# RaghuvirJonnagiri/LatticeBoltzmannSimulations

Measured on AMD Instinct MI355X. Metric: MLUPS (million lattice updates/sec) D2Q9 MRT cavity, higher is better.
Workload: dtype f32

## Files before the change

latticeboltzmannsimulations_amd/csrc/lbm_device.hpp:

```cpp
#pragma once
#include <hip/hip_runtime.h>

#include <type_traits>

#include "lbm_rheology.hpp"

namespace lbm {

constexpr int Q = 9;
constexpr int GH = 4;
constexpr int GHY = 10;

__host__ __device__ constexpr int cxk(int k) { return k == 1 || k == 5 || k == 8 ? 1 : (k == 3 || k == 6 || k == 7 ? -1 : 0); }
__host__ __device__ constexpr int cyk(int k) { return k == 2 || k == 5 || k == 6 ? 1 : (k == 4 || k == 7 || k == 8 ? -1 : 0); }

enum { SEM_PY = 0, SEM_GPU = 1, SEM_BB = 2, SEM_SOLID = 3 };
constexpr bool sem_is_bb(int sem) { return sem == SEM_BB || sem == SEM_SOLID; }
enum { C_SRT = 0, C_TRT = 1, C_MRT = 2,
       C_MRT_FAST = 3,
       C_SRT_FAST = 4,
       C_TRT_FAST = 5,
       C_SRT_PROM = 6, C_TRT_PROM = 7, C_MRT_PROM = 8 };
constexpr bool coll_is_mrt(int c) { return c == C_MRT || c == C_MRT_FAST || c == C_MRT_PROM; }
constexpr bool coll_is_fast(int c) { return c == C_MRT_FAST || c == C_SRT_FAST || c == C_TRT_FAST; }
constexpr bool coll_is_prom(int c) { return c == C_SRT_PROM || c == C_TRT_PROM || c == C_MRT_PROM; }

template <typename R>
struct Relax {
    R uLB, w_nu, w_m, w_e, w_eps, w_q;
};

typedef float f32x2 __attribute__((ext_vector_type(2)));
template <typename T> struct ScalarOf { typedef T type; };
template <> struct ScalarOf<f32x2> { typedef float type; };

template <int SEM>
__device__ __forceinline__ bool in_window(int k, int x, int gy, int X, int Y) {
    const int cx = cxk(k), cy = cyk(k);
    bool ok = true;
    if (sem_is_bb(SEM)) {
        return true;
    } else if (SEM == SEM_PY) {
        if (cx > 0) ok = ok && (x >= 1) && (x <= X - 2);
        if (cx < 0) ok = ok && (x <= X - 3);
        if (cy > 0) ok = ok && (gy <= Y - 3);
        if (cy < 0) ok = ok && (gy >= 1) && (gy <= Y - 2);
    } else {
        if (cx > 0) ok = ok && (x >= 1);
        if (cx < 0) ok = ok && (x <= X - 2);
        if (cy > 0) ok = ok && (gy <= Y - 2);
        if (cy < 0) ok = ok && (gy >= 1);
    }
    return ok;
}

template <typename T>
__device__ __forceinline__ T cu_of(int k, T ux, T uy) {
    switch (k) {
        case 1: return ux;
        case 2: return uy;
        case 3: return -ux;
        case 4: return -uy;
        case 5: return ux + uy;
        case 6: return -ux + uy;
        case 7: return -ux + -uy;
        case 8: return ux + -uy;
        default: return T{};
    }
}
template <typename R>
__device__ __forceinline__ R weight(int k) {
    return k == 0 ? (R)(4.0 / 9.0) : (k < 5 ? (R)(1.0 / 9.0) : (R)(1.0 / 36.));
}
template <bool FAST> __device__ __forceinline__ float div_(float a, float b) { return FAST ? a * __builtin_amdgcn_rcpf(b) : a / b; }
__device__ __forceinline__ double rcp_nr(double b) {
    double r = __builtin_amdgcn_rcp(b);
    r = __builtin_fma(__builtin_fma(-b, r, 1.0), r, r);
    r = __builtin_fma(__builtin_fma(-b, r, 1.0), r, r);
    return r;
}
template <bool FAST> __device__ __forceinline__ double div_(double a, double b) { return FAST ? a * rcp_nr(b) : a / b; }
template <bool FAST> __device__ __forceinline__ f32x2 div_(f32x2 a, f32x2 b) {
    return FAST ? a * f32x2{__builtin_amdgcn_rcpf(b.x), __builtin_amdgcn_rcpf(b.y)} : a / b;
}
template <bool FAST> __device__ __forceinline__ float sqrt_(float a) { return FAST ? __builtin_amdgcn_sqrtf(a) : sqrtf(a); }
template <bool FAST> __device__ __forceinline__ double sqrt_(double a) {
    if (!FAST) return sqrt(a);
    if (a <= 0.0) return 0.0;
    double y = __builtin_amdgcn_rsq(a);
    y = y * __builtin_fma(-0.5 * a * y, y, 1.5);
    y = y * __builtin_fma(-0.5 * a * y, y, 1.5);
    const double g = a * y;
    return __builtin_fma(__builtin_fma(-g, g, a), 0.5 * y, g);
}
template <bool FAST> __device__ __forceinline__ f32x2 sqrt_(f32x2 a) {
    return FAST ? f32x2{__builtin_amdgcn_sqrtf(a.x), __builtin_amdgcn_sqrtf(a.y)} : f32x2{sqrtf(a.x), sqrtf(a.y)};
}

template <typename F> __device__ __forceinline__ float lanes(F f, float a, float b) { return f(a, b); }
template <typename F> __device__ __forceinline__ f32x2 lanes(F f, f32x2 a, f32x2 b) { return f32x2{f(a.x, b.x), f(a.y, b.y)}; }
template <typename F> __device__ __forceinline__ float lanes(F f, float a, float b, float c) { return f(a, b, c); }
template <typename F> __device__ __forceinline__ f32x2 lanes(F f, f32x2 a, f32x2 b, f32x2 c) { return f32x2{f(a.x, b.x, c.x), f(a.y, b.y, c.y)}; }

__device__ __forceinline__ float feq_prom(float rt, float cu, float usqr) {
    const double c = (double)cu;
    return (float)((double)rt * (((1. + 3.0 * c) + (4.5 * c) * c) - 1.5 * (double)usqr));
}
__device__ __forceinline__ f32x2 feq_prom(f32x2 rt, f32x2 cu, f32x2 usqr) {
    return f32x2{feq_prom(rt.x, cu.x, usqr.x), feq_prom(rt.y, cu.y, usqr.y)};
}

template <typename T, bool PROM = false>
__device__ __forceinline__ void equ(T rho, T ux, T uy, T (&feq)[Q]) {
    typedef typename ScalarOf<T>::type S;
    const T usqr = ux * ux + uy * uy;
    if constexpr (PROM) {
#pragma unroll
        for (int k = 0; k < Q; ++k) feq[k] = feq_prom(rho * weight<S>(k), cu_of<T>(k, ux, uy), usqr);
        return;
    }
    const T c = (S)1.5 * usqr;
#pragma unroll
    for (int k = 0; k < Q; ++k) {
        const T cu = cu_of<T>(k, ux, uy);
        feq[k] = (rho * weight<S>(k)) * ((((S)1. + (S)3.0 * cu) + ((S)4.5 * cu) * cu) - c);
    }
}

template <typename R, bool FAST = false, int SEM = SEM_GPU>
__device__ __forceinline__ void macros(const R (&f)[Q], int x, int gy, int X, int Y, R uLB, R& rho, R& ux, R& uy) {
    rho = ((((((((f[0] + f[1]) + f[2]) + f[3]) + f[4]) + f[5]) + f[6]) + f[7]) + f[8]);
    ux = div_<FAST>((((((f[1] - f[3]) + f[5]) - f[6]) - f[7]) + f[8]), rho);
    uy = div_<FAST>((((((f[2] - f[4]) + f[5]) + f[6]) - f[7]) - f[8]), rho);
    if (sem_is_bb(SEM)) return;
    if (x == 0 || x == X - 1 || gy == Y - 1) { ux = (R)0; uy = (R)0; }
    if (gy == 0) {
        rho = ((f[0] + f[1]) + f[3]) + (R)2. * ((f[2] + f[5]) + f[6]);
        ux = uLB; uy = (R)0;
    }
}

__device__ __forceinline__ float fma_(float a, float b, float c) { return __builtin_fmaf(a, b, c); }
__device__ __forceinline__ double fma_(double a, double b, double c) { return __builtin_fma(a, b, c); }
__device__ __forceinline__ f32x2 fma_(f32x2 a, f32x2 b, f32x2 c) { return __builtin_elementwise_fma(a, b, c); }

template <typename T, int COLL, bool WM = false>
__device__ __forceinline__ void collide(const T (&f)[Q], T rho, const T (&feq)[Q],
                                        const Relax<typename ScalarOf<T>::type>& w, T w_nu, T (&out)[Q], bool lid = false, T w_m = T{}) {
    typedef typename ScalarOf<T>::type R;
    if (COLL == C_SRT || COLL == C_SRT_FAST || COLL == C_SRT_PROM) {
#pragma unroll
        for (int k = 0; k < Q; ++k) out[k] = f[k] - w_nu * (f[k] - feq[k]);
    } else if (COLL == C_TRT || COLL == C_TRT_FAST || COLL == C_TRT_PROM) {
        T fp[Q], fm[Q], ep[Q], em[Q];
        constexpr int pa[4] = {2, 5, 6, 1}, pb[4] = {4, 7, 8, 3};
#pragma unroll
        for (int i = 0; i < 4; ++i) {
            const int a = pa[i], b = pb[i];
            fp[a] = (R)0.5 * (f[a] + f[b]); fp[b] = fp[a];
            fm[a] = (R)0.5 * (f[a] - f[b]); fm[b] = -fm[a];
            ep[a] = (R)0.5 * (feq[a] + feq[b]); ep[b] = ep[a];
            em[a] = (R)0.5 * (feq[a] - feq[b]); em[b] = -em[a];
        }
        fp[0] = f[0]; fm[0] = T{}; ep[0] = feq[0]; em[0] = T{};
#pragma unroll
        for (int k = 0; k < Q; ++k) {
            if constexpr (WM) out[k] = (f[k] - w_nu * (fp[k] - ep[k])) - w_m * (fm[k] - em[k]);
            else out[k] = (f[k] - w_nu * (fp[k] - ep[k])) - w.w_m * (fm[k] - em[k]);
        }
    } else if (COLL == C_MRT_FAST) {
        const T a13 = f[1] + f[3], d13 = f[1] - f[3], a24 = f[2] + f[4], d24 = f[2] - f[4];
        const T a57 = f[5] + f[7], d57 = f[5] - f[7], a68 = f[6] + f[8], d68 = f[6] - f[8];
        const T sa = a13 + a24, sd = a57 + a68, dm = d57 - d68, dp = d57 + d68;
        const T r = (f[0] + sa) + sd;
        const T jx = d13 + dm, jy = d24 + dp;
        const T f04 = (R)4 * f[0];
        T e = fma_(T((R)2), sd, -sa) - f04;
        T eps = fma_(T((R)-2), sa, f04 + sd);
        T qx = fma_(T((R)-2), d13, dm), qy = fma_(T((R)-2), d24, dp);
        T pxx = a13 - a24, pxy = a57 - a68;
        const T jx2 = jx * jx, jy2 = jy * jy, j23 = (R)3 * (jx2 + jy2);
        const T rq = lid ? rho : r;
        e = fma_(T(-w.w_e), e - fma_(T((R)-2), rq, j23), e);
        eps = fma_(T(-w.w_eps), eps - fma_(T((R)9), jx2 * jy2, rq - j23), eps);
        qx = fma_(T(-w.w_q), qx - jx * fma_(T((R)3), jx2, T((R)-1)), qx);
        qy = fma_(T(-w.w_q), qy - jy * fma_(T((R)3), jy2, T((R)-1)), qy);
        pxx = fma_(-w_nu, pxx - (jx2 - jy2), pxx);
        pxy = fma_(-w_nu, fma_(-jx, jy, pxy), pxy);
        const R a9 = (R)(1.0 / 9), a36 = (R)(1.0 / 36), a18 = (R)(1.0 / 18), a6 = (R)(1.0 / 6),
                a12 = (R)(1.0 / 12), a4 = (R)(1.0 / 4);
        const T r9 = a9 * r;
        out[0] = a9 * ((r - e) + eps);
        const T A = fma_(T(-a18), eps, fma_(T(-a36), e, r9)), D = fma_(T(a36), eps, fma_(T(a18), e, r9));
        const T Ap = fma_(T(a4), pxx, A), Am = fma_(T(-a4), pxx, A), Dp = fma_(T(a4), pxy, D), Dm = fma_(T(-a4), pxy, D);
        const T bx = a6 * (jx - qx), by = a6 * (jy - qy);
        const T X = fma_(T(a12), qx, a6 * jx), Y = fma_(T(a12), qy, a6 * jy);
        const T XpY = X + Y, XmY = X - Y;
        out[1] = Ap + bx; out[3] = Ap - bx;
        out[2] = Am + by; out[4] = Am - by;
        out[5] = Dp + XpY; out[7] = Dp - XpY;
        out[8] = Dm + XmY; out[6] = Dm - XmY;
    } else {
        T m[Q], meq[Q];
        const T c2 = T((R)2), cm2 = T((R)-2);
        m[0] = (((((((f[0] + f[1]) + f[2]) + f[3]) + f[4]) + f[5]) + f[6]) + f[7]) + f[8];
        m[1] = fma_(c2, f[8], fma_(c2, f[7], fma_(c2, f[6], fma_(c2, f[5], ((((R)-4 * f[0] - f[1]) - f[2]) - f[3]) - f[4]))));
        m[2] = (((fma_(cm2, f[4], fma_(cm2, f[3], fma_(cm2, f[2], fma_(cm2, f[1], (R)4 * f[0])))) + f[5]) + f[6]) + f[7]) + f[8];
        m[3] = ((((f[1] - f[3]) + f[5]) - f[6]) - f[7]) + f[8];
        m[4] = (((fma_(c2, f[3], (R)-2 * f[1]) + f[5]) - f[6]) - f[7]) + f[8];
        m[5] = ((((f[2] - f[4]) + f[5]) + f[6]) - f[7]) - f[8];
        m[6] = (((fma_(c2, f[4], (R)-2 * f[2]) + f[5]) + f[6]) - f[7]) - f[8];
        m[7] = ((f[1] - f[2]) + f[3]) - f[4];
        m[8] = ((f[5] - f[6]) + f[7]) - f[8];
        const T jx = m[3], jy = m[5];
        meq[0] = rho;
        meq[1] = fma_(cm2, rho, (R)3.0 * (jx * jx + jy * jy));
        meq[2] = ((R)-3.0 * (jx * jx + jy * jy) + rho) + (R)9.0 * (((jx * jx) * jy) * jy);
        meq[3] = m[3];
        meq[4] = -jx + (R)3.0 * ((jx * jx) * jx);
        meq[5] = m[5];
        meq[6] = -jy + (R)3.0 * ((jy * jy) * jy);
        meq[7] = jx * jx - jy * jy;
        meq[8] = jx * jy;
        if constexpr (COLL == C_MRT_PROM) {
            const T s = jx * jx + jy * jy, p4 = ((jx * jx) * jy) * jy, x3 = (jx * jx) * jx, y3 = (jy * jy) * jy;
            meq[1] = lanes([](float r, float a) { return (float)(-2.0 * (double)r + 3.0 * (double)a); }, rho, s);
            meq[2] = lanes([](float a, float r, float b) { return (float)((-3.0 * (double)a + (double)r) + 9.0 * (double)b); }, s, rho, p4);
            meq[4] = lanes([](float j, float a) { return (float)((double)(-j) + 3.0 * (double)a); }, jx, x3);
            meq[6] = lanes([](float j, float a) { return (float)((double)(-j) + 3.0 * (double)a); }, jy, y3);
        }
        m[1] = m[1] - w.w_e * (m[1] - meq[1]);
        m[2] = m[2] - w.w_eps * (m[2] - meq[2]);
        m[4] = m[4] - w.w_q * (m[4] - meq[4]);
        m[6] = m[6] - w.w_q * (m[6] - meq[6]);
        m[7] = m[7] - w_nu * (m[7] - meq[7]);
        m[8] = m[8] - w_nu * (m[8] - meq[8]);
        const R a9 = (R)(1.0 / 9), a36 = (R)(1.0 / 36), a18 = (R)(1.0 / 18), a6 = (R)(1.0 / 6),
                a12 = (R)(1.0 / 12), a4 = (R)(1.0 / 4);
        const T q4 = T(a4), qm4 = T(-a4);
        out[0] = (a9 * m[0] + -a9 * m[1]) + a9 * m[2];
        out[1] = fma_(q4, m[7], (((a9 * m[0] + -a36 * m[1]) + -a18 * m[2]) + a6 * m[3]) + -a6 * m[4]);
        out[2] = fma_(qm4, m[7], (((a9 * m[0] + -a36 * m[1]) + -a18 * m[2]) + a6 * m[5]) + -a6 * m[6]);
        out[3] = fma_(q4, m[7], (((a9 * m[0] + -a36 * m[1]) + -a18 * m[2]) + -a6 * m[3]) + a6 * m[4]);
        out[4] = fma_(qm4, m[7], (((a9 * m[0] + -a36 * m[1]) + -a18 * m[2]) + -a6 * m[5]) + a6 * m[6]);
        out[5] = fma_(q4, m[8], (((((a9 * m[0] + a18 * m[1]) + a36 * m[2]) + a6 * m[3]) + a12 * m[4]) + a6 * m[5]) + a12 * m[6]);
        out[6] = fma_(qm4, m[8], (((((a9 * m[0] + a18 * m[1]) + a36 * m[2]) + -a6 * m[3]) + -a12 * m[4]) + a6 * m[5]) + a12 * m[6]);
        out[7] = fma_(q4, m[8], (((((a9 * m[0] + a18 * m[1]) + a36 * m[2]) + -a6 * m[3]) + -a12 * m[4]) + -a6 * m[5]) + -a12 * m[6]);
        out[8] = fma_(qm4, m[8], (((((a9 * m[0] + a18 * m[1]) + a36 * m[2]) + a6 * m[3]) + a12 * m[4]) + -a6 * m[5]) + -a12 * m[6]);
    }
}

constexpr int K_QEQ = Q;
constexpr int K_RHO = Q + 1;

template <typename T>
__device__ __forceinline__ T diag_flux(const T (&f)[Q]) {
    return -f[8] + (f[7] + (-f[6] + f[5]));
}
template <typename T, int COLL, bool TURB, bool WM = false>
__device__ __forceinline__ void equ_collide(const T (&g)[Q], T rho, T ux, T uy, const Relax<typename ScalarOf<T>::type>& w, T w_nu, T (&out)[Q], T& q2,
                                            bool lid = false, T w_m = T{}) {
    typedef typename ScalarOf<T>::type R;
    if constexpr ((COLL == C_SRT_FAST && !(TURB && sizeof(R) == 4)) || COLL == C_TRT_FAST) {
        const T base = fma_(T((R)-1.5), fma_(uy, uy, ux * ux), T((R)1));
        const T orho = w_nu * rho, c1 = (R)1 - w_nu;
        const T r1 = (R)(1.0 / 9) * orho, r5 = (R)(1.0 / 36) * orho;
        out[0] = fma_((R)(4.0 / 9) * orho, base, c1 * g[0]);
        if constexpr (COLL == C_SRT_FAST) {
            auto pair = [&](T cu, T rw, const T& ga, const T& gb, T& oa, T& ob) {
                const T e = fma_((R)4.5 * cu, cu, base), o = (R)3 * cu;
                oa = fma_(rw, e + o, c1 * ga);
                ob = fma_(rw, e - o, c1 * gb);
            };
            pair(ux, r1, g[1], g[3], out[1], out[3]);
            pair(uy, r1, g[2], g[4], out[2], out[4]);
            pair(ux + uy, r5, g[5], g[7], out[5], out[7]);
            pair(ux - uy, r5, g[8], g[6], out[8], out[6]);
        } else {
            const auto wm = [&] { if constexpr (WM) return w_m; else return w.w_m; }();
            const T mrho = wm * rho, hp = (R)0.5 * w_nu;
            const T m1 = (R)(1.0 / 9) * mrho, m5 = (R)(1.0 / 36) * mrho;
            const auto hm = (R)0.5 * wm;
            auto pair = [&](T cu, T rp, T rm, const T& ga, const T& gb, T& oa, T& ob) {
                const T e = fma_((R)4.5 * cu, cu, base), o = (R)3 * cu;
                const T P = fma_(-rp, e, hp * (ga + gb)), M = fma_(-rm, o, hm * (ga - gb));
                oa = (ga - P) - M;
                ob = (gb - P) + M;
            };
            pair(ux, r1, m1, g[1], g[3], out[1], out[3]);
            pair(uy, r1, m1, g[2], g[4], out[2], out[4]);
            pair(ux + uy, r5, m5, g[5], g[7], out[5], out[7]);
            pair(ux - uy, r5, m5, g[8], g[6], out[8], out[6]);
        }
        if (TURB) q2 = rho * (ux * uy);
    } else if constexpr (COLL == C_MRT_FAST) {
        T fe[Q];
        collide<T, COLL>(g, rho, fe, w, w_nu, out, lid);
        if (TURB) q2 = rho * (ux * uy);
    } else {
        T fe[Q];
        if (!coll_is_mrt(COLL) || TURB) equ<T, coll_is_prom(COLL)>(rho, ux, uy, fe);
        if constexpr (WM) collide<T, COLL, true>(g, rho, fe, w, w_nu, out, false, w_m);
        else collide<T, COLL>(g, rho, fe, w, w_nu, out);
        if (TURB) q2 = diag_flux<T>(fe);
    }
}

__device__ __forceinline__ float real_abs(float x) { return fabsf(x); }
__device__ __forceinline__ double real_abs(double x) { return fabs(x); }
__device__ __forceinline__ f32x2 real_abs(f32x2 x) { return f32x2{fabsf(x.x), fabsf(x.y)}; }

template <typename T, bool FAST = false, bool PROM = false>
__device__ __forceinline__ T smagorinsky_tau(const T (&f)[Q], T qeq_prev, T rho_prev, typename ScalarOf<T>::type omega) {
    typedef typename ScalarOf<T>::type R;
    const R tau0 = (R)1.0 / omega;
    const T q = diag_flux<T>(f) - qeq_prev;
    if constexpr (PROM) {
        const R tt = tau0 * tau0;
        return lanes([tau0, tt](float qq, float rp) {
            return (float)(0.5 * ((double)tau0 + sqrt((double)tt + (((18 * 1.4142) * (double)0.025f) * (double)fabsf(qq)) / (double)rp)));
        }, q, rho_prev);
    }
    return (R)0.5 * (tau0 + sqrt_<FAST>(tau0 * tau0 + div_<FAST>(((R)(18 * 1.4142) * (R)0.025) * real_abs(q), rho_prev)));
}
template <typename T, bool FAST = false, bool PROM = false>
__device__ __forceinline__ T smagorinsky_omega(const T (&f)[Q], T qeq_prev, T rho_prev, typename ScalarOf<T>::type omega) {
    typedef typename ScalarOf<T>::type R;
    return div_<FAST>(T((R)1.0), smagorinsky_tau<T, FAST, PROM>(f, qeq_prev, rho_prev, omega));
}

template <typename T, bool FAST = false, typename W = typename ScalarOf<T>::type>
__device__ __forceinline__ T subgrid_tau(const T (&f)[Q], T rho, T ux, T uy, W omega, typename ScalarOf<T>::type k) {
    typedef typename ScalarOf<T>::type R;
    const W tau0 = (R)1.0 / omega;
    const T sxx = ((((f[1] + f[3]) + f[5]) + f[6]) + f[7]) + f[8];
    const T syy = ((((f[2] + f[4]) + f[5]) + f[6]) + f[7]) + f[8];
    const T sxy = ((f[5] - f[6]) + f[7]) - f[8];
    const T r3 = rho * (R)(1.0 / 3), jx = rho * ux;
    const T pxx = sxx - (r3 + jx * ux);
    const T pyy = syy - (r3 + (rho * uy) * uy);
    const T pxy = sxy - jx * uy;
    const T n = sqrt_<FAST>((pxx * pxx + (R)2 * (pxy * pxy)) + pyy * pyy);
    return (R)0.5 * (tau0 + sqrt_<FAST>(tau0 * tau0 + div_<FAST>(k * n, rho)));
}
template <typename T, bool FAST = false, typename W = typename ScalarOf<T>::type>
__device__ __forceinline__ T subgrid_omega(const T (&f)[Q], T rho, T ux, T uy, W omega, typename ScalarOf<T>::type k) {
    typedef typename ScalarOf<T>::type R;
    return div_<FAST>(T((R)1.0), subgrid_tau<T, FAST, W>(f, rho, ux, uy, omega, k));
}

template <typename R>
struct Rheo {
    const R* tab;
    R inv_dg;
// ... 711 lines not shown
```

latticeboltzmannsimulations_amd/csrc/lbm_stream.hpp:

```cpp
#pragma once
#include "lbm_kernels.hpp"

constexpr int ST_WAVES = 16;
constexpr int ST_NT = ST_WAVES * 64;
constexpr int ST_MAX_S = ST_WAVES / 2;
constexpr int ST_LDS_BYTES = ST_WAVES * 9 * 1024;

__device__ __forceinline__ int dpp_from_lower(int v) { return __builtin_amdgcn_update_dpp(v, v, 0x138, 0xf, 0xf, false); }
__device__ __forceinline__ int dpp_from_upper(int v) { return __builtin_amdgcn_update_dpp(v, v, 0x130, 0xf, 0xf, false); }
__device__ __forceinline__ float lane_lower(float v) { return __builtin_bit_cast(float, dpp_from_lower(__builtin_bit_cast(int, v))); }
__device__ __forceinline__ float lane_upper(float v) { return __builtin_bit_cast(float, dpp_from_upper(__builtin_bit_cast(int, v))); }
__device__ __forceinline__ double lane_lower(double v) {
    const long long b = __builtin_bit_cast(long long, v);
    const unsigned lo = (unsigned)dpp_from_lower((int)(unsigned)b), hi = (unsigned)dpp_from_lower((int)(unsigned)(b >> 32));
    return __builtin_bit_cast(double, (long long)(((unsigned long long)hi << 32) | lo));
}
__device__ __forceinline__ double lane_upper(double v) {
    const long long b = __builtin_bit_cast(long long, v);
    const unsigned lo = (unsigned)dpp_from_upper((int)(unsigned)b), hi = (unsigned)dpp_from_upper((int)(unsigned)(b >> 32));
    return __builtin_bit_cast(double, (long long)(((unsigned long long)hi << 32) | lo));
}

__device__ __forceinline__ float lane_lower_e(float v, float edge) {
    return __builtin_bit_cast(float, __builtin_amdgcn_update_dpp(__builtin_bit_cast(int, edge), __builtin_bit_cast(int, v), 0x138, 0xf, 0xf, false));
}
__device__ __forceinline__ float lane_upper_e(float v, float edge) {
    return __builtin_bit_cast(float, __builtin_amdgcn_update_dpp(__builtin_bit_cast(int, edge), __builtin_bit_cast(int, v), 0x130, 0xf, 0xf, false));
}
__device__ __forceinline__ double lane_lower_e(double v, double edge) {
    const long long b = __builtin_bit_cast(long long, v), e = __builtin_bit_cast(long long, edge);
    const unsigned lo = (unsigned)__builtin_amdgcn_update_dpp((int)(unsigned)e, (int)(unsigned)b, 0x138, 0xf, 0xf, false);
    const unsigned hi = (unsigned)__builtin_amdgcn_update_dpp((int)(unsigned)(e >> 32), (int)(unsigned)(b >> 32), 0x138, 0xf, 0xf, false);
    return __builtin_bit_cast(double, (long long)(((unsigned long long)hi << 32) | lo));
}
__device__ __forceinline__ double lane_upper_e(double v, double edge) {
    const long long b = __builtin_bit_cast(long long, v), e = __builtin_bit_cast(long long, edge);
    const unsigned lo = (unsigned)__builtin_amdgcn_update_dpp((int)(unsigned)e, (int)(unsigned)b, 0x130, 0xf, 0xf, false);
    const unsigned hi = (unsigned)__builtin_amdgcn_update_dpp((int)(unsigned)(e >> 32), (int)(unsigned)(b >> 32), 0x130, 0xf, 0xf, false);
    return __builtin_bit_cast(double, (long long)(((unsigned long long)hi << 32) | lo));
}
template <typename R, int V>
__device__ __forceinline__ typename VecT<R, V>::type shift_from_lower_e(typename VecT<R, V>::type own, R edge) {
    typename VecT<R, V>::type r;
    r[0] = lane_lower_e(own[V - 1], edge);
#pragma unroll
    for (int c = 1; c < V; ++c) r[c] = own[c - 1];
    return r;
}
template <typename R, int V>
__device__ __forceinline__ typename VecT<R, V>::type shift_from_upper_e(typename VecT<R, V>::type own, R edge) {
    typename VecT<R, V>::type r;
#pragma unroll
    for (int c = 0; c < V - 1; ++c) r[c] = own[c + 1];
    r[V - 1] = lane_upper_e(own[0], edge);
    return r;
}

template <typename R, int V>
__device__ __forceinline__ typename VecT<R, V>::type shift_from_lower(typename VecT<R, V>::type own) {
    typename VecT<R, V>::type r;
    r[0] = lane_lower(own[V - 1]);
#pragma unroll
    for (int c = 1; c < V; ++c) r[c] = own[c - 1];
    return r;
}
template <typename R, int V>
__device__ __forceinline__ typename VecT<R, V>::type shift_from_upper(typename VecT<R, V>::type own) {
    typename VecT<R, V>::type r;
#pragma unroll
    for (int c = 0; c < V - 1; ++c) r[c] = own[c + 1];
    r[V - 1] = lane_upper(own[0]);
    return r;
}

__host__ __device__ constexpr int stream_rim(int S, int V) { return (S + V - 1) / V * V; }

#ifdef LBM_EXPERIMENT_NO_BARRIER
__device__ __forceinline__ void lds_barrier() { asm volatile("s_waitcnt lgkmcnt(0)" ::: "memory"); }
#else
__device__ __forceinline__ void lds_barrier() { asm volatile("s_waitcnt lgkmcnt(0)\n\ts_barrier" ::: "memory"); }
#endif

template <typename R, int V, bool PROM = false>
__device__ __forceinline__ void wall_row_rules(typename VecT<R, V>::type (&in)[Q], typename VecT<R, V>::type& rw, bool lid, R uLB, bool wl, bool wr,
                                               R& kl, R& kr) {
    typedef typename VecT<R, V>::type T;
    if (lid) {
        const T ux = T(uLB), uy = T((R)0);
        const T cq = (R)1.5 * (ux * ux + uy * uy);
        auto fek = [&](int k) {
            const T cu = cu_of<T>(k, ux, uy);
            if constexpr (PROM) {
                const T rt = rw * weight<R>(k), usqr = ux * ux + uy * uy;
                T fe;
#pragma unroll
                for (int c = 0; c < V; ++c) fe[c] = feq_prom(rt[c], cu[c], usqr[c]);
                return fe;
            } else {
                return (rw * weight<R>(k)) * ((((R)1. + (R)3.0 * cu) + ((R)4.5 * cu) * cu) - cq);
            }
        };
        if (wl) {
            const R g7 = kl;
            in[1][0] = (fek(1)[0] - fek(3)[0]) + in[3][0];
            in[5][0] = (fek(5)[0] - fek(7)[0]) + g7;
            in[8][0] = (fek(8)[0] - fek(6)[0]) + in[6][0];
        }
        if (wr) {
            const R g8 = kr;
            in[3][V - 1] = (-fek(1)[V - 1] + fek(3)[V - 1]) + in[1][V - 1];
            in[6][V - 1] = (-fek(8)[V - 1] + fek(6)[V - 1]) + g8;
            in[7][V - 1] = (-fek(5)[V - 1] + fek(7)[V - 1]) + in[5][V - 1];
        }
        in[4] = (-fek(2) + fek(4)) + in[2];
        in[7] = (-fek(5) + fek(7)) + in[5];
        in[8] = (-fek(6) + fek(8)) + in[6];
        if (wl) kl = in[7][0];
        if (wr) kr = in[8][V - 1];
        rw = ((in[0] + in[1]) + in[3]) + (R)2. * ((in[2] + in[5]) + in[6]);
    } else {
        if (wl) {
            const R g6 = kl;
            in[1][0] = (R)0 + in[3][0];
            in[5][0] = (R)0 + in[7][0];
            in[8][0] = (R)0 + g6;
        }
        if (wr) {
            const R g5 = kr;
            in[3][V - 1] = (R)0 + in[1][V - 1];
            in[6][V - 1] = (R)0 + in[8][V - 1];
            in[7][V - 1] = (R)0 + g5;
        }
        in[2] = (R)0 + in[4];
        in[5] = (R)0 + in[7];
        in[6] = (R)0 + in[8];
        if (wl) kl = in[6][0];
        if (wr) kr = in[5][V - 1];
    }
}

template <typename R, int V, bool WALLS>
__device__ __forceinline__ void build_in(typename VecT<R, V>::type (&in)[Q], typename VecT<R, V>::type o0, typename VecT<R, V>::type o1,
                                         typename VecT<R, V>::type o3, typename VecT<R, V>::type u2, typename VecT<R, V>::type u5,
                                         typename VecT<R, V>::type u6, typename VecT<R, V>::type d4, typename VecT<R, V>::type d7,
                                         typename VecT<R, V>::type d8) {
    in[0] = o0;
    in[2] = u2;
    in[4] = d4;
    if (WALLS) {
        in[1] = shift_from_lower_e<R, V>(o1, (R)0 + o3[1]);
        in[5] = shift_from_lower_e<R, V>(u5, (R)0 + d7[1]);
        in[8] = shift_from_lower_e<R, V>(d8, (R)0 + u6[1]);
        in[3] = shift_from_upper_e<R, V>(o3, (R)0 + o1[V - 2]);
        in[6] = shift_from_upper_e<R, V>(u6, (R)0 + d8[V - 2]);
        in[7] = shift_from_upper_e<R, V>(d7, (R)0 + u5[V - 2]);
    } else {
        in[1] = shift_from_lower<R, V>(o1);
        in[5] = shift_from_lower<R, V>(u5);
        in[8] = shift_from_lower<R, V>(d8);
        in[3] = shift_from_upper<R, V>(o3);
        in[6] = shift_from_upper<R, V>(u6);
        in[7] = shift_from_upper<R, V>(d7);
    }
}

template <typename R, int COLL, bool TURB, bool WALLS = false, bool SLAB = false>
__device__ __forceinline__ void stream_segment(const R* __restrict__ src, R* __restrict__ dst, const Geo& geo, const Relax<R>& w, R* __restrict__ lds,
                                               int S, int xs, int ya, int yb, int xe, int own_lo = 0, int own_hi = 0) {
    constexpr int V = 16 / (int)sizeof(R), ROW = 64 * V;
    typedef typename VecT<R, V>::type T;
    const int wv = __builtin_amdgcn_readfirstlane((int)(threadIdx.x >> 6)), lane = threadIdx.x & 63;
    const int q = ((wv & 7) << 1) | (wv >> 3);
    const int RV = stream_rim(S, V) / V;
    const bool wall_lo = WALLS && (!SLAB || geo.y0 == 0), wall_hi = WALLS && (!SLAB || geo.y0 + geo.ny == geo.NY);
    const int y_first = wall_lo ? max(ya - (S - 1), 0) : ya - (S - 1);
    const int y_end = wall_hi ? min(yb + (S - 1), geo.ny) : yb + (S - 1);
    const int y_lid = wall_lo ? 0 : -(1 << 30), y_bot = wall_hi ? geo.ny - 1 : -(1 << 30);
    const int nb = y_end - y_first;
    const int x0 = xs + lane * V;
    const bool lane_in = x0 < geo.nx;
    const bool lane_out = WALLS ? (x0 >= own_lo && x0 < own_hi) : (lane >= RV && lane < 64 - RV && x0 < xe);
    const bool wl = WALLS && x0 == 0, wr = WALLS && x0 + V == geo.nx;
    const bool side_strip = WALLS && (xs == 0 || xs + ROW >= geo.nx);
    const bool narrow = WALLS && xs + ROW > geo.nx;
    R* const slot_mine = lds + (q * 9) * ROW;
    R* const up_mine = slot_mine + lane * V;
    const R* const up_below = lds + (((q + 1) & (ST_WAVES - 1)) * 9) * ROW + lane * V;
    const R* const down_above = lds + (((q + ST_WAVES - 1) & (ST_WAVES - 1)) * 9 + 3) * ROW + lane * V;

    T in[Q], outv[Q], hq, hr;
#ifdef LBM_EXP_NO_HBM
    auto row_base = [&](const R* p, int k, int y) { return (const char*)(p + ((long long)k * geo.plane + (long long)((y & 63) + GHY) * geo.row)); };
#else
    auto row_base = [&](const R* p, int k, int y) { return (const char*)(p + ((long long)k * geo.plane + (long long)(y + GHY) * geo.row)); };
#endif
    const unsigned lane_off = (unsigned)(GH + x0) * (unsigned)sizeof(R);
    auto cell = [&](const char* base, int dx) {
        unsigned off = lane_off;
        asm volatile("" : "+v"(off));
        return (const R*)(base + (off + (unsigned)(dx * (int)sizeof(R))));
    };
    const unsigned lane_off_ld = WALLS ? (unsigned)(GH + min(x0, max(geo.nx - V, 0))) * (unsigned)sizeof(R) : lane_off;
    auto cell_ld = [&](const char* base, int dx) {
        unsigned off = lane_off_ld;
        asm volatile("" : "+v"(off));
        return (const R*)(base + (off + (unsigned)(dx * (int)sizeof(R))));
    };
    auto load_row = [&](int y, bool exists) {
        if (WALLS) {
            if (exists) {
#pragma unroll
                for (int k = 0; k < Q; ++k) in[k] = vload<R, V, false>(cell_ld(row_base(src, k, y + cyk(k)), -cxk(k)), cxk(k) == 0);
                if (TURB) {
                    hq = vload<R, V, false>(cell_ld(row_base(src, K_QEQ, y), 0), true);
                    hr = vload<R, V, false>(cell_ld(row_base(src, K_RHO, y), 0), true);
                }
            } else {
#pragma unroll
                for (int k = 0; k < Q; ++k) in[k] = T{};
                hq = hr = T{};
            }
            return;
        }
        if (!lane_in || !exists) return;
#pragma unroll
        for (int k = 0; k < Q; ++k) in[k] = vload<R, V, false>(cell(row_base(src, k, y + cyk(k)), -cxk(k)), cxk(k) == 0);
        if (TURB) {
            hq = vload<R, V, false>(cell(row_base(src, K_QEQ, y), 0), true);
            hr = vload<R, V, false>(cell(row_base(src, K_RHO, y), 0), true);
        }
    };
    auto post = [&](int level, bool up, bool down) __attribute__((always_inline)) {
        R* const dn = up_mine + (3 + (level & 1) * 3) * ROW;
        const T p2 = outv[2], p5 = outv[5], p6 = outv[6], p4 = outv[4], p7 = outv[7], p8 = outv[8];
#ifdef LBM_EXP_NO_LDS
        if (geo.nx < 0)
#endif
        if (up) {
            *reinterpret_cast<T*>(up_mine) = p2;
            *reinterpret_cast<T*>(up_mine + ROW) = p5;
            *reinterpret_cast<T*>(up_mine + 2 * ROW) = p6;
        }
#ifdef LBM_EXP_NO_LDS
        if (geo.nx < 0)
#endif
        if (down) {
            *reinterpret_cast<T*>(dn) = p4;
            *reinterpret_cast<T*>(dn + ROW) = p7;
            *reinterpret_cast<T*>(dn + 2 * ROW) = p8;
        }
    };
    auto block = [&](int b, auto wrow_tag) __attribute__((always_inline)) {
        constexpr bool WROW = decltype(wrow_tag)::value;
        const int y = y_first + b;
        const bool wrow = WALLS && WROW, lid = WALLS && WROW && y == 0;
        R* const st = slot_mine + (lid ? 0 : 3 * ROW);
        auto update = [&](bool first) {
            int kind = 0;
            T rw = T{};
            R kl = (R)0, kr = (R)0;
            if (WALLS) {
                if constexpr (WROW) {
                    if (first) {
                        if (lid) rw = vload<R, V, false>(cell_ld(row_base(src, 0, -1), 0), true);
                        kl = lid ? in[7][0] : in[6][0];
                        kr = lid ? in[8][V - 1] : in[5][V - 1];
                    } else {
                        if (lid) rw = *reinterpret_cast<const T*>(st + lane * V);
                        kl = st[ROW + lane];
                        kr = st[2 * ROW + lane];
                    }
                    wall_row_rules<R, V, coll_is_prom(COLL)>(in, rw, lid, w.uLB, wl, wr, kl, kr);
                    kind = lid ? 1 : 2;
                } else if (side_strip && (first || narrow)) {
                    if (wl && first) { in[1][0] = (R)0 + in[3][0]; in[5][0] = (R)0 + in[7][0]; in[8][0] = (R)0 + in[6][0]; }
                    if (wr) { in[3][V - 1] = (R)0 + in[1][V - 1]; in[6][V - 1] = (R)0 + in[8][V - 1]; in[7][V - 1] = (R)0 + in[5][V - 1]; }
                }
            }
#ifdef LBM_EXP_NO_COLLIDE
#pragma unroll
            for (int k = 0; k < Q; ++k) outv[k] = in[k];
#else
            collide_vec<R, COLL, V, TURB>(in, w, outv, hq, hr, wl && kind == 0, wr && kind == 0, kind);
#endif
            if constexpr (WALLS && WROW) {
                if (lid) *reinterpret_cast<T*>(st + lane * V) = rw;
                st[ROW + lane] = kl;
                st[2 * ROW + lane] = kr;
            }
        };
        const bool up = !lid, down = !(wrow && !lid);
        update(true);
        if (S > 1) post(1, up, down);
        lds_barrier();
        lds_barrier();
        for (int l = 1; l < S; ++l) {
            const R* const dn = down_above + (l & 1) * 3 * ROW;
#ifdef LBM_EXP_NO_LDS
            build_in<R, V, WALLS>(in, outv[0], outv[1], outv[3], outv[2], outv[5], outv[6], outv[4], outv[7], outv[8]);
#else
            build_in<R, V, WALLS>(in, outv[0], outv[1], outv[3], *reinterpret_cast<const T*>(up_below), *reinterpret_cast<const T*>(up_below + ROW),
                                  *reinterpret_cast<const T*>(up_below + 2 * ROW), *reinterpret_cast<const T*>(dn), *reinterpret_cast<const T*>(dn + ROW),
                                  *reinterpret_cast<const T*>(dn + 2 * ROW));
#endif
            update(false);
            if (l + 1 < S) {
                post(l + 1, up, down);
                lds_barrier();
                lds_barrier();
            }
        }
        {
            const T hq_done = hq, hr_done = hr;
            T rw_done = T{};
            R kl_done = (R)0, kr_done = (R)0;
            if (WALLS && wrow) {
                if (lid) rw_done = *reinterpret_cast<const T*>(st + lane * V);
                kl_done = st[ROW + lane];
                kr_done = st[2 * ROW + lane];
            }
            if (lane_out && y >= ya && y < yb) {
#pragma unroll
                for (int k = 0; k < Q; ++k) vstore<R, V, false>(const_cast<R*>(cell(row_base(dst, k, y), 0)), outv[k]);
                if (TURB) {
                    vstore<R, V, false>(const_cast<R*>(cell(row_base(dst, K_QEQ, y), 0)), hq_done);
                    vstore<R, V, false>(const_cast<R*>(cell(row_base(dst, K_RHO, y), 0)), hr_done);
                }
                if (WALLS && wrow) {
                    if (lid) {
                        vstore<R, V, false>(const_cast<R*>(cell(row_base(dst, 0, -1), 0)), rw_done);
                        if (wl) *const_cast<R*>(cell(row_base(dst, 7, -1), 1)) = kl_done;
                        if (wr) *const_cast<R*>(cell(row_base(dst, 8, -1), V - 2)) = kr_done;
                    } else {
                        if (wl) *const_cast<R*>(cell(row_base(dst, 6, geo.ny), 1)) = kl_done;
                        if (wr) *const_cast<R*>(cell(row_base(dst, 5, geo.ny), V - 2)) = kr_done;
                    }
                }
            }
            if (S > 1) lds_barrier();
            load_row(y_first + b + ST_WAVES, b + ST_WAVES < nb);
            if (S > 1) lds_barrier();
        }
        for (int i = 2 * S; i < ST_WAVES; ++i) lds_barrier();
    };
#pragma unroll
    for (int k = 0; k < Q; ++k) in[k] = T{};
    hq = T{}; hr = T{};
    for (int i = 0; i < q; ++i) lds_barrier();
    load_row(y_first + q, q < nb);
    for (int b = q; b < nb; b += ST_WAVES) {
        const int y = y_first + b;
        if (WALLS && (SLAB ? (y == y_lid || y == y_bot) : (y == 0 || y == geo.ny - 1))) block(b, std::true_type{});
        else block(b, std::false_type{});
    }
}

template <typename R, int COLL, int SEM, bool TURB>
__global__ __launch_bounds__(ST_NT) void k_stream(const R* __restrict__ src, R* __restrict__ dst, Geo geo, Relax<R> w, int S, int F, int xe, int ye,
                                                  int nstrips, int H, FramePtrs<R> fp, int nframe, int nsegx, int nsegy, int seg, int use_lds,
                                                  int lo, int hi, int bands, int xcd_bands) {
    __shared__ __align__(16) R lds[ST_LDS_BYTES / sizeof(R)];
    if ((int)blockIdx.x < nframe) {
        frame_passes<R, COLL, SEM, TURB, ST_NT>(fp, 0, geo, w, F, S, nsegx, nsegy, lo, hi, (int)blockIdx.x, seg, use_lds ? lds : nullptr, bands);
        return;
    }
    constexpr int V = 16 / (int)sizeof(R);
    int b = blockIdx.x - nframe;
    if (xcd_bands) {
        const int per = ((int)gridDim.x - nframe) >> 3;
        if (b < (per << 3)) b = (b & 7) * per + (b >> 3);
    }
    const int strip = b % nstrips, sy = b / nstrips;
    const int R_ = stream_rim(S, V);
    const int xs = F - R_ + strip * (64 * V - 2 * R_);
    int ya, yb;
    if (bands) {
        const bool top = (bands & 1) && sy == 0;
        if (top) { ya = -(lo > 0 ? lo - 1 : 0); yb = F; }
        else { ya = geo.ny - F; yb = geo.ny + (hi > 0 ? hi - 1 : 0); }
    } else {
        ya = F + sy * H; yb = min(ye, ya + H);
    }
    if (ya >= yb) return;
    stream_segment<R, COLL, TURB>(src, dst, geo, w, lds, S, xs, ya, yb, xe);
}

__host__ __device__ constexpr int stream_walls_strips(int nx, int S, int V) {
    return nx <= 64 * V ? 1 : (nx - 64 * V + (64 * V - 2 * stream_rim(S, V)) - 1) / (64 * V - 2 * stream_rim(S, V)) + 1;
}
template <int V>
__device__ __forceinline__ void walls_strip(const Geo& geo, int S, int strip, int nstrips, int& xs, int& own_lo, int& own_hi) {
    const int R_ = stream_rim(S, V), TXu = 64 * V - 2 * R_;
    xs = min(strip * TXu, max(geo.nx - 64 * V, 0));
    own_lo = strip == 0 ? 0 : strip * TXu + R_;
    own_hi = strip == nstrips - 1 ? geo.nx : (strip + 1) * TXu + R_;
}

template <typename R, int COLL, bool TURB>
__global__ __launch_bounds__(ST_NT) void k_stream_walls(const R* __restrict__ src, R* __restrict__ dst, Geo geo, Relax<R> w, int S, int nstrips, int H,
                                                        int xcd_bands) {
    __shared__ __align__(16) R lds[ST_LDS_BYTES / sizeof(R)];
    constexpr int V = 16 / (int)sizeof(R);
    const int b = xcd_bands ? xcd_band(blockIdx.x, gridDim.x) : (int)blockIdx.x;
    const int strip = b % nstrips, sy = b / nstrips;
    int xs, own_lo, own_hi;
    walls_strip<V>(geo, S, strip, nstrips, xs, own_lo, own_hi);
    const int ya = sy * H, yb = min(geo.ny, ya + H);
    if (ya >= yb) return;
    stream_segment<R, COLL, TURB, true>(src, dst, geo, w, lds, S, xs, ya, yb, 0, own_lo, own_hi);
}
template <typename R, int COLL, bool TURB>
__global__ __launch_bounds__(ST_NT) void k_stream_walls_slab(const R* __restrict__ src, R* __restrict__ dst, Geo geo, Relax<R> w, int S, int nstrips, int H,
                                                             int xcd_bands, int ybeg, int yend, int bands, int lo, int hi, int F) {
    __shared__ __align__(16) R lds[ST_LDS_BYTES / sizeof(R)];
    constexpr int V = 16 / (int)sizeof(R), W = 64 * V;
    int b = blockIdx.x;
    if (xcd_bands) {
        const int per = (int)gridDim.x >> 3;
        if (b < (per << 3)) b = (b & 7) * per + (b >> 3);
    }
    const int strip = b % nstrips, sy = b / nstrips;
    const int R_ = stream_rim(S, V), TXu = W - 2 * R_;
    const int xs = min(strip * TXu, max(geo.nx - W, 0));
    const int own_lo = strip == 0 ? 0 : strip * TXu + R_;
    const int own_hi = strip == nstrips - 1 ? geo.nx : (strip + 1) * TXu + R_;
    int ya, yb;
    if (bands) {
        const bool top = (bands & 1) && sy == 0;
        if (top) { ya = -(lo > 0 ? lo - 1 : 0); yb = F; }
        else { ya = geo.ny - F; yb = geo.ny + (hi > 0 ? hi - 1 : 0); }
    } else {
        ya = ybeg + sy * H; yb = min(yend, ya + H);
    }
    if (ya >= yb) return;
    stream_segment<R, COLL, TURB, true, true>(src, dst, geo, w, lds, S, xs, ya, yb, 0, own_lo, own_hi);
}

constexpr int SP_MAX_WAVES = 12;
constexpr int SP_NT = SP_MAX_WAVES * 64;

constexpr int SP_MAX_S = SP_MAX_WAVES - 2;
constexpr int SP_SLOTS = 12;
constexpr int SP_LDS_BYTES = SP_MAX_WAVES * SP_SLOTS * 1024;

template <typename R, int COLL, bool TURB>
__device__ __forceinline__ void stream_pairs_segment(const R* __restrict__ src, R* __restrict__ dst, const Geo& geo, const Relax<R>& w, R* __restrict__ lds,
                                                     int S, int xs, int ya, int yb, int own_lo, int own_hi) {
    constexpr int V = 16 / (int)sizeof(R), ROW = 64 * V;
    typedef typename VecT<R, V>::type T;
    const int W = (int)(blockDim.x >> 6);
    const int wv = __builtin_amdgcn_readfirstlane((int)(threadIdx.x >> 6)), lane = threadIdx.x & 63;
    const int y_first = max(ya - (S - 1), 0), y_end = min(yb + (S - 1), geo.ny);
    const int nb = y_end - y_first, npairs = (nb + 1) >> 1;
    const int x0 = xs + lane * V;
    const bool lane_out = x0 >= own_lo && x0 < own_hi;
    const bool wl = x0 == 0, wr = x0 + V == geo.nx;
    const bool side_strip = xs == 0 || xs + ROW >= geo.nx;
    const bool narrow = xs + ROW > geo.nx;
    R* const slot_mine = lds + (wv * SP_SLOTS) * ROW;
    R* const post_mine = slot_mine + lane * V;
    const R* const up_below = lds + (((wv + 1 == W ? 0 : wv + 1)) * SP_SLOTS) * ROW + lane * V;
    const R* const down_above = lds + (((wv == 0 ? W - 1 : wv - 1)) * SP_SLOTS + 3) * ROW + lane * V;
// ... 197 lines not shown
```

Measured before the change: 381,100.

## Pair cells into packed f32x2 MRT collide with swizzled lane layout

```diff
diff --git a/latticeboltzmannsimulations_amd/csrc/lbm_device.hpp b/latticeboltzmannsimulations_amd/csrc/lbm_device.hpp
--- a/latticeboltzmannsimulations_amd/csrc/lbm_device.hpp
+++ b/latticeboltzmannsimulations_amd/csrc/lbm_device.hpp
@@ -144,6 +144,41 @@
 __device__ __forceinline__ double fma_(double a, double b, double c) { return __builtin_fma(a, b, c); }
 __device__ __forceinline__ f32x2 fma_(f32x2 a, f32x2 b, f32x2 c) { return __builtin_elementwise_fma(a, b, c); }
 
+template <typename T>
+__device__ __forceinline__ void mrt_fast_rest(T f0, T a13, T d13, T a24, T d24, T a57, T d57, T a68, T d68, T rho,
+                                              const Relax<typename ScalarOf<T>::type>& w, T w_nu, T (&out)[Q], bool lid) {
+    typedef typename ScalarOf<T>::type R;
+    const T sa = a13 + a24, sd = a57 + a68, dm = d57 - d68, dp = d57 + d68;
+    const T r = (f0 + sa) + sd;
+    const T jx = d13 + dm, jy = d24 + dp;
+    const T f04 = (R)4 * f0;
+    T e = fma_(T((R)2), sd, -sa) - f04;
+    T eps = fma_(T((R)-2), sa, f04 + sd);
+    T qx = fma_(T((R)-2), d13, dm), qy = fma_(T((R)-2), d24, dp);
+    T pxx = a13 - a24, pxy = a57 - a68;
+    const T jx2 = jx * jx, jy2 = jy * jy, j23 = (R)3 * (jx2 + jy2);
+    const T rq = lid ? rho : r;
+    e = fma_(T(-w.w_e), e - fma_(T((R)-2), rq, j23), e);
+    eps = fma_(T(-w.w_eps), eps - fma_(T((R)9), jx2 * jy2, rq - j23), eps);
+    qx = fma_(T(-w.w_q), qx - jx * fma_(T((R)3), jx2, T((R)-1)), qx);
+    qy = fma_(T(-w.w_q), qy - jy * fma_(T((R)3), jy2, T((R)-1)), qy);
+    pxx = fma_(-w_nu, pxx - (jx2 - jy2), pxx);
+    pxy = fma_(-w_nu, fma_(-jx, jy, pxy), pxy);
+    const R a9 = (R)(1.0 / 9), a36 = (R)(1.0 / 36), a18 = (R)(1.0 / 18), a6 = (R)(1.0 / 6),
+            a12 = (R)(1.0 / 12), a4 = (R)(1.0 / 4);
+    const T r9 = a9 * r;
+    out[0] = a9 * ((r - e) + eps);
+    const T A = fma_(T(-a18), eps, fma_(T(-a36), e, r9)), D = fma_(T(a36), eps, fma_(T(a18), e, r9));
+    const T Ap = fma_(T(a4), pxx, A), Am = fma_(T(-a4), pxx, A), Dp = fma_(T(a4), pxy, D), Dm = fma_(T(-a4), pxy, D);
+    const T bx = a6 * (jx - qx), by = a6 * (jy - qy);
+    const T X = fma_(T(a12), qx, a6 * jx), Y = fma_(T(a12), qy, a6 * jy);
+    const T XpY = X + Y, XmY = X - Y;
+    out[1] = Ap + bx; out[3] = Ap - bx;
+    out[2] = Am + by; out[4] = Am - by;
+    out[5] = Dp + XpY; out[7] = Dp - XpY;
+    out[8] = Dm + XmY; out[6] = Dm - XmY;
+}
+
 template <typename T, int COLL, bool WM = false>
 __device__ __forceinline__ void collide(const T (&f)[Q], T rho, const T (&feq)[Q],
                                         const Relax<typename ScalarOf<T>::type>& w, T w_nu, T (&out)[Q], bool lid = false, T w_m = T{}) {
@@ -171,35 +206,7 @@
     } else if (COLL == C_MRT_FAST) {
         const T a13 = f[1] + f[3], d13 = f[1] - f[3], a24 = f[2] + f[4], d24 = f[2] - f[4];
         const T a57 = f[5] + f[7], d57 = f[5] - f[7], a68 = f[6] + f[8], d68 = f[6] - f[8];
-        const T sa = a13 + a24, sd = a57 + a68, dm = d57 - d68, dp = d57 + d68;
-        const T r = (f[0] + sa) + sd;
-        const T jx = d13 + dm, jy = d24 + dp;
-        const T f04 = (R)4 * f[0];
-        T e = fma_(T((R)2), sd, -sa) - f04;
-        T eps = fma_(T((R)-2), sa, f04 + sd);
-        T qx = fma_(T((R)-2), d13, dm), qy = fma_(T((R)-2), d24, dp);
-        T pxx = a13 - a24, pxy = a57 - a68;
-        const T jx2 = jx * jx, jy2 = jy * jy, j23 = (R)3 * (jx2 + jy2);
-        const T rq = lid ? rho : r;
-        e = fma_(T(-w.w_e), e - fma_(T((R)-2), rq, j23), e);
-        eps = fma_(T(-w.w_eps), eps - fma_(T((R)9), jx2 * jy2, rq - j23), eps);
-        qx = fma_(T(-w.w_q), qx - jx * fma_(T((R)3), jx2, T((R)-1)), qx);
-        qy = fma_(T(-w.w_q), qy - jy * fma_(T((R)3), jy2, T((R)-1)), qy);
-        pxx = fma_(-w_nu, pxx - (jx2 - jy2), pxx);
-        pxy = fma_(-w_nu, fma_(-jx, jy, pxy), pxy);
-        const R a9 = (R)(1.0 / 9), a36 = (R)(1.0 / 36), a18 = (R)(1.0 / 18), a6 = (R)(1.0 / 6),
-                a12 = (R)(1.0 / 12), a4 = (R)(1.0 / 4);
-        const T r9 = a9 * r;
-        out[0] = a9 * ((r - e) + eps);
-        const T A = fma_(T(-a18), eps, fma_(T(-a36), e, r9)), D = fma_(T(a36), eps, fma_(T(a18), e, r9));
-        const T Ap = fma_(T(a4), pxx, A), Am = fma_(T(-a4), pxx, A), Dp = fma_(T(a4), pxy, D), Dm = fma_(T(-a4), pxy, D);
-        const T bx = a6 * (jx - qx), by = a6 * (jy - qy);
-        const T X = fma_(T(a12), qx, a6 * jx), Y = fma_(T(a12), qy, a6 * jy);
-        const T XpY = X + Y, XmY = X - Y;
-        out[1] = Ap + bx; out[3] = Ap - bx;
-        out[2] = Am + by; out[4] = Am - by;
-        out[5] = Dp + XpY; out[7] = Dp - XpY;
-        out[8] = Dm + XmY; out[6] = Dm - XmY;
+        mrt_fast_rest<T>(f[0], a13, d13, a24, d24, a57, d57, a68, d68, rho, w, w_nu, out, lid);
     } else {
         T m[Q], meq[Q];
         const T c2 = T((R)2), cm2 = T((R)-2);
diff --git a/latticeboltzmannsimulations_amd/csrc/lbm_stream.hpp b/latticeboltzmannsimulations_amd/csrc/lbm_stream.hpp
--- a/latticeboltzmannsimulations_amd/csrc/lbm_stream.hpp
+++ b/latticeboltzmannsimulations_amd/csrc/lbm_stream.hpp
@@ -164,11 +164,51 @@
     }
 }
 
+__device__ __forceinline__ f32x2 pk_add_x0(f32x2 a, f32x2 b) { f32x2 r; asm("v_pk_add_f32 %0, %1, %2 op_sel:[1,0] op_sel_hi:[0,1]" : "=v"(r) : "v"(a), "v"(b)); return r; }
+__device__ __forceinline__ f32x2 pk_sub_x0(f32x2 a, f32x2 b) { f32x2 r; asm("v_pk_add_f32 %0, %1, %2 op_sel:[1,0] op_sel_hi:[0,1] neg_lo:[0,1] neg_hi:[0,1]" : "=v"(r) : "v"(a), "v"(b)); return r; }
+__device__ __forceinline__ f32x2 pk_add_x1(f32x2 a, f32x2 b) { f32x2 r; asm("v_pk_add_f32 %0, %1, %2 op_sel:[0,1] op_sel_hi:[1,0]" : "=v"(r) : "v"(a), "v"(b)); return r; }
+__device__ __forceinline__ f32x2 pk_sub_x1(f32x2 a, f32x2 b) { f32x2 r; asm("v_pk_add_f32 %0, %1, %2 op_sel:[0,1] op_sel_hi:[1,0] neg_lo:[0,1] neg_hi:[0,1]" : "=v"(r) : "v"(a), "v"(b)); return r; }
+
+template <typename T, typename R>
+__device__ __forceinline__ void paired_update(T (&outv)[Q], T u2, T u5, T u6, T d4, T d7, T d8, const Relax<R>& w, bool side_strip, bool wl, bool wr) {
+    static_assert(std::is_same<T, VecT<float, 4>::type>::value && std::is_same<R, float>::value, "fp32, four cells per lane");
+    const T o0 = outv[0], o1 = outv[1], o3 = outv[3];
+    float e1 = lane_lower(o1.w), e5 = lane_lower(u5.w), e8 = lane_lower(d8.w);
+    float w3 = lane_upper(o3.x), w6 = lane_upper(u6.x), w7 = lane_upper(d7.x);
+    if (side_strip) {
+        auto zero_plus = [](float x) __attribute__((always_inline)) { float r; asm("v_add_f32 %0, 0, %1" : "=v"(r) : "v"(x)); return r; };
+        asm volatile("");
+        const float l1 = zero_plus(o3.z), l5 = zero_plus(d7.z), l8 = zero_plus(u6.z);
+        const float r3 = zero_plus(o1.y), r6 = zero_plus(d8.y), r7 = zero_plus(u5.y);
+        e1 = wl ? l1 : e1; e5 = wl ? l5 : e5; e8 = wl ? l8 : e8;
+        w3 = wr ? r3 : w3; w6 = wr ? r6 : w6; w7 = wr ? r7 : w7;
+    }
+    const f32x2 x1 = f32x2{o1.z, e1}, x5 = f32x2{u5.z, e5}, x8 = f32x2{d8.z, e8};
+    const f32x2 x3 = f32x2{w3, o3.y}, x6 = f32x2{w6, u6.y}, x7 = f32x2{w7, d7.y};
+    const f32x2 w_nu = (f32x2)(w.w_nu);
+    f32x2 out0[Q], out1[Q];
+    mrt_fast_rest<f32x2>(o0.xy, pk_add_x0(x1, o3.zw), pk_sub_x0(x1, o3.zw), u2.xy + d4.xy, u2.xy - d4.xy, pk_add_x0(x5, d7.zw), pk_sub_x0(x5, d7.zw),
+                         pk_add_x1(u6.zw, x8), pk_sub_x1(u6.zw, x8), f32x2(0.f), w, w_nu, out0, false);
+    mrt_fast_rest<f32x2>(o0.zw, pk_add_x1(o1.xy, x3), pk_sub_x1(o1.xy, x3), u2.zw + d4.zw, u2.zw - d4.zw, pk_add_x1(u5.xy, x7), pk_sub_x1(u5.xy, x7),
+                         pk_add_x0(x6, d8.xy), pk_sub_x0(x6, d8.xy), f32x2(0.f), w, w_nu, out1, false);
+#pragma unroll
+    for (int k = 0; k < Q; ++k) { outv[k].xy = out0[k]; outv[k].zw = out1[k]; }
+}
+
 template <typename R, int COLL, bool TURB, bool WALLS = false, bool SLAB = false>
 __device__ __forceinline__ void stream_segment(const R* __restrict__ src, R* __restrict__ dst, const Geo& geo, const Relax<R>& w, R* __restrict__ lds,
                                                int S, int xs, int ya, int yb, int xe, int own_lo = 0, int own_hi = 0) {
     constexpr int V = 16 / (int)sizeof(R), ROW = 64 * V;
     typedef typename VecT<R, V>::type T;
+#ifdef LBM_EXP_NO_COLLIDE
+    constexpr bool PAIRED = false;
+#else
+    constexpr bool PAIRED = sizeof(R) == 4 && COLL == C_MRT_FAST && !TURB;
+#endif
+    auto pswap = [](T v) __attribute__((always_inline)) {
+        if constexpr (PAIRED) return T{v[0], v[2], v[1], v[3]};
+        else return v;
+    };
     const int wv = __builtin_amdgcn_readfirstlane((int)(threadIdx.x >> 6)), lane = threadIdx.x & 63;
     const int q = ((wv & 7) << 1) | (wv >> 3);
     const int RV = stream_rim(S, V) / V;
@@ -230,9 +270,11 @@
             hr = vload<R, V, false>(cell(row_base(src, K_RHO, y), 0), true);
         }
     };
-    auto post = [&](int level, bool up, bool down) __attribute__((always_inline)) {
+    auto post = [&](int level, bool up, bool down, auto swap_tag) __attribute__((always_inline)) {
         R* const dn = up_mine + (3 + (level & 1) * 3) * ROW;
-        const T p2 = outv[2], p5 = outv[5], p6 = outv[6], p4 = outv[4], p7 = outv[7], p8 = outv[8];
+        constexpr bool SWAP = decltype(swap_tag)::value;
+        const T p2 = SWAP ? pswap(outv[2]) : outv[2], p5 = SWAP ? pswap(outv[5]) : outv[5], p6 = SWAP ? pswap(outv[6]) : outv[6],
+                p4 = SWAP ? pswap(outv[4]) : outv[4], p7 = SWAP ? pswap(outv[7]) : outv[7], p8 = SWAP ? pswap(outv[8]) : outv[8];
 #ifdef LBM_EXP_NO_LDS
         if (geo.nx < 0)
 #endif
@@ -290,24 +332,42 @@
             }
         };
         const bool up = !lid, down = !(wrow && !lid);
+        constexpr bool PROW = PAIRED && !WROW;
+        typedef std::integral_constant<bool, PAIRED && WROW> swap_tag;
         update(true);
-        if (S > 1) post(1, up, down);
+        if constexpr (PROW) {
+            if (S > 1) {
+#pragma unroll
+                for (int k = 0; k < Q; ++k) outv[k] = pswap(outv[k]);
+            }
+        }
+        if (S > 1) post(1, up, down, swap_tag{});
         lds_barrier();
         lds_barrier();
         for (int l = 1; l < S; ++l) {
             const R* const dn = down_above + (l & 1) * 3 * ROW;
 #ifdef LBM_EXP_NO_LDS
-            build_in<R, V, WALLS>(in, outv[0], outv[1], outv[3], outv[2], outv[5], outv[6], outv[4], outv[7], outv[8]);
+            const T n2 = outv[2], n5 = outv[5], n6 = outv[6], n4 = outv[4], n7 = outv[7], n8 = outv[8];
 #else
-            build_in<R, V, WALLS>(in, outv[0], outv[1], outv[3], *reinterpret_cast<const T*>(up_below), *reinterpret_cast<const T*>(up_below + ROW),
-                                  *reinterpret_cast<const T*>(up_below + 2 * ROW), *reinterpret_cast<const T*>(dn), *reinterpret_cast<const T*>(dn + ROW),
-                                  *reinterpret_cast<const T*>(dn + 2 * ROW));
+            const T n2 = *reinterpret_cast<const T*>(up_below), n5 = *reinterpret_cast<const T*>(up_below + ROW), n6 = *reinterpret_cast<const T*>(up_below + 2 * ROW),
+                    n4 = *reinterpret_cast<const T*>(dn), n7 = *reinterpret_cast<const T*>(dn + ROW), n8 = *reinterpret_cast<const T*>(dn + 2 * ROW);
 #endif
-            update(false);
+            if constexpr (PROW) {
+                paired_update<T, R>(outv, n2, n5, n6, n4, n7, n8, w, side_strip, wl, wr);
+            } else {
+                build_in<R, V, WALLS>(in, outv[0], outv[1], outv[3], pswap(n2), pswap(n5), pswap(n6), pswap(n4), pswap(n7), pswap(n8));
+                update(false);
+            }
             if (l + 1 < S) {
-                post(l + 1, up, down);
+                post(l + 1, up, down, swap_tag{});
                 lds_barrier();
                 lds_barrier();
+            }
+        }
+        if constexpr (PROW) {
+            if (S > 1) {
+#pragma unroll
+                for (int k = 0; k < Q; ++k) outv[k] = pswap(outv[k]);
             }
         }
         {
```

Result: slower. 366,800 (-3.8%).
